# jandrewrfarrell/RUFUS

Hardware: AMD Instinct MI355X
Metric: reads/sec through k-mer count+filter at k=25 (higher is better)
Workload: dtype u64; 1 GPU; synthetic 30x WGS trio (BASELINE configs[2]): genome 3100000000 bp, 620000000/620000000/620000000 x 150 bp reads per sample, on each of 1 GPU(s) 19 resident blocks of the subject (92 GB of packed reads in HBM, generated on the device in 2.7 s), 1000 SNVs, seed 12345, k=25, -s 8G -L 2, MinCov 5, MaxHashDepth 1200, MinQ 15, thresh 1; 2 minimizer-shard pass(es) per step (per-shard (pos,key)-sorted re; parallelism=read-block shard x1, mutant_kmers=24567, pulled_pairs=11560, passes=2, hbm_total=309220868096, hbm_free_at_start=308400881664, resident_read_bytes=92219805240, read_blocks=compact, run_map_budget_bytes=39836680704, checked=False, hbm_mapped_bytes=271656681472

## Files before the change

include/rufus_hip.h:

```cpp
#ifndef RUFUS_HIP_H
#define RUFUS_HIP_H

#include <stddef.h>
#include <stdint.h>

#ifdef __cplusplus
extern "C" {
#endif

#define RFX_OK 0
#define RFX_E_NODEVICE (-1)
#define RFX_E_INVAL (-2)
#define RFX_E_NOMEM (-3)
#define RFX_E_FULL (-4)
#define RFX_E_HIP (-5)
#define RFX_E_MIXEDCASE (-6)
#define RFX_E_RANGE (-7)
#define RFX_E_FORMAT (-8)

#define RFX_HISTO_BINS 10002

typedef struct rfx_ctx rfx_ctx;
typedef struct rfx_reads rfx_reads;
typedef struct rfx_table rfx_table;
// ... 183 lines not shown
rfx_records* rfx_records_load(rfx_ctx*, int k, int lsize, const uint64_t* cols, const void* payload, uint64_t n,
                              int counter_len);
rfx_records* rfx_records_load_fd(rfx_ctx*, int k, int lsize, const uint64_t* cols, int fd, uint64_t offset, uint64_t n,
                                 int counter_len);
rfx_records* rfx_records_from_dev(rfx_ctx*, int k, int lsize, const uint64_t* cols, const uint64_t* d_keys,
                                  const uint32_t* d_counts, uint64_t n);
const uint64_t* rfx_records_dev_keys(const rfx_records*);
const uint32_t* rfx_records_dev_counts(const rfx_records*);
const uint64_t* rfx_records_dev_pos(const rfx_records*);
int rfx_records_histo(const rfx_records*, uint64_t* histo );
int rfx_records_verify(const rfx_records*, uint32_t min_count, uint32_t max_count, uint64_t out[4]);
int rfx_records_checksum(const rfx_records*, uint64_t out[2]);
void rfx_records_free(rfx_records*);

int rfx_merge_unique(rfx_ctx*, const rfx_records* const* files, int n_files, uint32_t min_count, uint64_t* keys_out,
                     uint32_t* counts_out, uint64_t cap, uint64_t* n_out);
int rfx_query(const rfx_records* db, const uint64_t* keys, uint64_t n, uint32_t* counts_out);
int rfx_unique_to_subject(rfx_ctx*, const rfx_records* subject, const rfx_records* const* others, int n_others,
                          uint32_t min_count, uint32_t min_cov, uint32_t max_cov, uint64_t* keys_out,
                          uint32_t* counts_out, uint64_t cap, uint64_t* n_out);
rfx_records* rfx_records_subtract(rfx_ctx*, const rfx_records* a, const rfx_records* const* others, int n_others,
                                  uint32_t min_count, uint32_t max_count);

typedef struct rfx_binned rfx_binned;
typedef struct rfx_candidates rfx_candidates;
rfx_binned* rfx_count_finish_binned(rfx_table*, uint64_t lower, uint64_t upper, uint64_t* histo );
uint64_t rfx_binned_size(const rfx_binned*);
int rfx_binned_bits(const rfx_binned*);
void rfx_binned_free(rfx_binned*);
rfx_candidates* rfx_binned_strike(rfx_ctx*, rfx_binned* subject, const rfx_binned* control, uint32_t min_count,
                                  uint32_t max_count);
int rfx_binned_strike_stats(const rfx_ctx*, uint64_t out[2]);
int rfx_leaf_variant(const rfx_ctx*, int out[2]);
int rfx_candidates_strike(rfx_candidates*, const rfx_binned* control);
uint64_t rfx_candidates_size(const rfx_candidates*);
int rfx_candidates_get(const rfx_candidates*, uint64_t* keys_out);
int rfx_candidates_get_counts(const rfx_candidates*, uint32_t* counts_out);
int rfx_candidates_strike_records(rfx_candidates*, const rfx_records* exclude);
void rfx_candidates_free(rfx_candidates*);
int rfx_binned_get(const rfx_binned*, uint64_t* keys_out, uint32_t* counts_out, uint32_t* bins_out, uint64_t* at_out,
                   uint64_t cap, uint64_t* n_out);
int rfx_binned_checksum(const rfx_binned*, uint64_t out[2]);
int rfx_binned_verify(const rfx_binned*, uint64_t lower, uint64_t upper, uint64_t out[5]);
int rfx_binned_query(const rfx_binned*, const uint64_t* canonical_keys, uint64_t n, uint32_t* counts_out);
const uint64_t* rfx_binned_dev_keys(const rfx_binned*);
const uint32_t* rfx_binned_dev_counts(const rfx_binned*);

rfx_set* rfx_set_build(rfx_ctx*, const uint64_t* fwd_keys, uint64_t n, int k);
uint64_t rfx_set_size(const rfx_set*);
void rfx_set_free(rfx_set*);
int rfx_filter(rfx_set*, const rfx_reads*, int thresh, int last_base_skipped, uint32_t* hits_out,
               uint64_t* hitmask_out, uint64_t* n_hit_reads);
int rfx_filter_many(rfx_set*, const rfx_reads* const* blocks, int n, int thresh, int last_base_skipped,
                    uint64_t* const* hitmask_out, uint64_t* n_hit_reads);

#define RFX_SELECT_READS 0
#define RFX_SELECT_PAIRS 1
rfx_reads* rfx_reads_select(rfx_ctx*, const rfx_reads* src, const uint64_t* hitmask , int mode);
int rfx_reads_origin(const rfx_reads*, uint32_t* block_out, uint32_t* read_out);
rfx_reads* rfx_filter_pull(rfx_set*, const rfx_reads* const* blocks, int n, int thresh, int last_base_skipped, int mode,
                           uint64_t* const* hitmask_out, uint64_t* n_hit_reads);

typedef struct rfx_model_params {
  double sc, stdev, factor, skew, power;
} rfx_model_params;
int rfx_model_residuals(rfx_ctx*, const int64_t* histo, uint32_t n, const rfx_model_params* cand, int n_cand,
// ... 22 lines not shown
```

rufus_amd/capi.py:

```python
from __future__ import annotations

import ctypes as C
import os
import sys

import numpy as np

_HERE = os.path.dirname(os.path.abspath(__file__))
LIB_PATH = os.environ.get("RFX_LIB") or os.path.join(_HERE, "librufus_hip.so")

HISTO_BINS = 10002
PACK_COUNT, PACK_FILTER = 1, 2
COUNT_AUTO, COUNT_TABLE, COUNT_P2L, COUNT_MSP = 0, 1, 2, 3
E_FULL, E_RANGE, E_MIXEDCASE = -4, -7, -6
E_INVAL, E_FORMAT = -2, -8
SELECT_READS, SELECT_PAIRS = 0, 1

u8p, u32p, u64p = C.POINTER(C.c_uint8), C.POINTER(C.c_uint32), C.POINTER(C.c_uint64)

SIGNATURES = {
    "rfx_version": (C.c_char_p, []),
    "rfx_strerror": (C.c_char_p, [C.c_int]),
    "rfx_last_error": (C.c_char_p, []),
    "rfx_jf_matrix": (C.c_int, [C.c_int, C.c_int, u64p]),
    "rfx_jf_pos": (C.c_uint64, [u64p, C.c_int, C.c_int, C.c_uint64]),
    "rfx_pack_words": (C.c_uint64, [u64p, C.c_uint32]),
    "rfx_pack_reads": (C.c_int, [C.c_char_p, C.c_char_p, u64p, C.c_uint32, C.c_int, C.c_int, u64p, u32p, u32p, u32p,
                                 u32p]),
    "rfx_pack_spans": (C.c_int, [C.c_void_p, u64p, u32p, u64p, C.c_uint32, C.c_int, C.c_int, u64p, u32p, u32p, u32p, u32p]),
    "rfx_hashlist_keys": (C.c_long, [C.c_char_p, C.c_size_t, C.c_int, C.c_int, u64p, C.c_size_t]),
    "rfx_jhash_header": (C.c_long, [C.c_int, C.c_int, u64p, C.c_int, C.c_int, C.c_int, C.POINTER(C.c_char_p),
                                    C.c_char_p, C.c_size_t]),
    "rfx_open": (C.c_void_p, [C.c_int, C.c_size_t]),
    "rfx_close": (None, [C.c_void_p]),
    "rfx_sync": (C.c_int, [C.c_void_p]),
    "rfx_host_alloc": (C.c_void_p, [C.c_size_t]),
    "rfx_host_alloc_lazy": (C.c_void_p, [C.c_size_t]),
    "rfx_host_pin": (C.c_int, [C.c_void_p]),
    "rfx_host_cpus": (C.c_uint, []),
    "rfx_host_free": (None, [C.c_void_p]),
    "rfx_stream": (C.c_void_p, [C.c_void_p]),
    "rfx_mem_stats": (C.c_int, [C.c_void_p, u64p, u64p, u64p]),
    "rfx_memcpy_dev": (C.c_int, [C.c_void_p, C.c_void_p, C.c_void_p, C.c_size_t]),
    "rfx_prof_enable": (C.c_int, [C.c_void_p, C.c_int]),
    "rfx_prof_filter": (C.c_int, [C.c_void_p, C.c_char_p]),
    "rfx_prof_reset": (C.c_int, [C.c_void_p]),
    "rfx_prof_query": (C.c_int, [C.c_void_p, C.c_char_p, C.POINTER(C.c_double), u64p]),
    "rfx_prof_names": (C.c_int, [C.c_void_p, C.c_char_p, C.c_size_t]),
    "rfx_reads_device_bytes": (C.c_uint64, [C.c_void_p]),
    "rfx_records_subtract": (C.c_void_p, [C.c_void_p, C.c_void_p, C.POINTER(C.c_void_p), C.c_int, C.c_uint32, C.c_uint32]),
    "rfx_count_finish_binned": (C.c_void_p, [C.c_void_p, C.c_uint64, C.c_uint64, u64p]),
    "rfx_binned_size": (C.c_uint64, [C.c_void_p]),
    "rfx_binned_bits": (C.c_int, [C.c_void_p]),
    "rfx_binned_free": (None, [C.c_void_p]),
    "rfx_binned_strike": (C.c_void_p, [C.c_void_p, C.c_void_p, C.c_void_p, C.c_uint32, C.c_uint32]),
    "rfx_binned_strike_stats": (C.c_int, [C.c_void_p, u64p]),
    "rfx_leaf_variant": (C.c_int, [C.c_void_p, C.POINTER(C.c_int)]),
    "rfx_candidates_strike": (C.c_int, [C.c_void_p, C.c_void_p]),
    "rfx_candidates_size": (C.c_uint64, [C.c_void_p]),
    "rfx_candidates_get": (C.c_int, [C.c_void_p, u64p]),
    "rfx_candidates_free": (None, [C.c_void_p]),
    "rfx_candidates_get_counts": (C.c_int, [C.c_void_p, u32p]),
    "rfx_candidates_strike_records": (C.c_int, [C.c_void_p, C.c_void_p]),
    "rfx_binned_get": (C.c_int, [C.c_void_p, u64p, u32p, u32p, u64p, C.c_uint64, u64p]),
    "rfx_binned_checksum": (C.c_int, [C.c_void_p, u64p]),
    "rfx_binned_verify": (C.c_int, [C.c_void_p, C.c_uint64, C.c_uint64, u64p]),
    "rfx_binned_query": (C.c_int, [C.c_void_p, u64p, C.c_uint64, u32p]),
    "rfx_binned_dev_keys": (C.c_void_p, [C.c_void_p]),
    "rfx_binned_dev_counts": (C.c_void_p, [C.c_void_p]),
    "rfx_reads_upload": (C.c_void_p, [C.c_void_p, u64p, u32p, u32p, u32p, u32p, C.c_uint32]),
    "rfx_reads_free": (None, [C.c_void_p]),
    "rfx_reads_count": (C.c_uint32, [C.c_void_p]),
    "rfx_reads_bases": (C.c_uint64, [C.c_void_p]),
    "rfx_reads_words": (C.c_uint64, [C.c_void_p]),
    "rfx_reads_get": (C.c_int, [C.c_void_p, u64p, u32p, u32p, u32p, u32p]),
    "rfx_tile_plan": (C.c_int, [C.c_uint64, C.c_int, C.c_uint32, u64p, u32p]),
    "rfx_reads_tile": (C.c_void_p, [C.c_void_p, C.c_void_p, C.c_int, C.c_uint32]),
    "rfx_reads_select": (C.c_void_p, [C.c_void_p, C.c_void_p, u64p, C.c_int]),
    "rfx_reads_origin": (C.c_int, [C.c_void_p, u32p, u32p]),
    "rfx_filter_pull": (C.c_void_p, [C.c_void_p, C.POINTER(C.c_void_p), C.c_int, C.c_int, C.c_int, C.c_int, C.POINTER(u64p), u64p]),
    "rfx_synth_reads": (C.c_void_p, [C.c_void_p, C.c_void_p, C.c_uint64, C.c_uint32, C.c_int, C.c_int]),
    "rfx_text_open": (C.c_void_p, [C.c_void_p, C.c_uint64]),
    "rfx_text_close": (None, [C.c_void_p]),
    "rfx_text_room": (C.c_uint64, [C.c_void_p]),
    "rfx_text_bytes": (C.c_uint64, [C.c_void_p]),
    "rfx_text_append": (C.c_long, [C.c_void_p, C.c_char_p, C.c_uint64]),
    "rfx_text_copied": (C.c_int, [C.c_void_p, C.c_long]),
    "rfx_text_wait": (C.c_int, [C.c_void_p, C.c_long]),
    "rfx_text_parse": (C.c_void_p, [C.c_void_p, C.c_int, C.c_int, C.POINTER(C.c_int)]),
    "rfx_text_fetch": (C.c_int, [C.c_void_p, C.c_char_p]),
# ... 968 lines not shown
    def counts(self, raw_keys=None) -> np.ndarray:
        c = np.zeros(len(self), np.uint32)
        _check(lib().rfx_candidates_get_counts(self._h, _p(c, u32p)), "rfx_candidates_get_counts")
        k = self._raw_keys() if raw_keys is None else raw_keys
        return c[k != np.uint64(0xFFFFFFFFFFFFFFFF)]

    def keys_counts(self):
        k = self._raw_keys()
        return k[k != np.uint64(0xFFFFFFFFFFFFFFFF)], self.counts(k)

    def free(self):
        if self._h:
            lib().rfx_candidates_free(self._h)
            self._h = None


def binned_strike(ctx: Context, subject: Binned, control, min_count: int = 0, max_count: int = 0xFFFFFFFF) -> Candidates:
    return Candidates(ctx, lib().rfx_binned_strike(ctx._h, subject._h, control._h if control is not None else None,
                                                   min_count, max_count))


def binned_strike_stats(ctx: Context) -> dict:
    o = np.zeros(2, dtype=np.uint64)
    _check(lib().rfx_binned_strike_stats(ctx._h, _p(o, u64p)), "rfx_binned_strike_stats")
    return {"units": int(o[0]), "deferred": int(o[1])}


def leaf_variant(ctx: Context) -> dict:
    o = np.zeros(2, dtype=np.int32)
    _check(lib().rfx_leaf_variant(ctx._h, o.ctypes.data_as(C.POINTER(C.c_int))), "rfx_leaf_variant")
    return {"kc": int(o[0]), "one": bool(o[1])}


OVL_SAM, OVL_CONTIG, OVL_REGION = 0, 1, 2


def overlap_score(ctx: Context, a: bytes, cands, min_pct: float, min_ovl: int, variant: int = OVL_SAM) -> np.ndarray:
    nb = len(cands)
    arr = (C.c_char_p * max(nb, 1))(*cands)
    lens = (C.c_int * max(nb, 1))(*[len(x) for x in cands])
    out = np.zeros((max(nb, 1), 5), dtype=np.int32)
    _check(lib().rfx_overlap_score(ctx._h, a, len(a), arr, lens, nb, min_pct, min_ovl, variant,
                                   out.ctypes.data_as(C.POINTER(C.c_int))), "rfx_overlap_score")
    return out[:nb]


class OvlPool:

    def __init__(self, ctx: Context, seqs):
        self.ctx, self.n = ctx, len(seqs)
        arr = (C.c_char_p * max(self.n, 1))(*seqs)
        lens = (C.c_int * max(self.n, 1))(*[len(s) for s in seqs])
        self._h = lib().rfx_ovl_pool_create(ctx._h, arr, lens, self.n)
        if not self._h:
            raise RufusError("rfx_ovl_pool_create failed: " + lib().rfx_last_error().decode())

    def set(self, i: int, seq: bytes):
        _check(lib().rfx_ovl_pool_set(self._h, i, seq, len(seq)), "rfx_ovl_pool_set")

    def score(self, cands, min_pct: float, min_ovl: int, variant: int = OVL_SAM, strands: int = 0, query: int | None = None,
              a_explicit: bytes | None = None) -> np.ndarray:
        if (query is None) == (a_explicit is None):
            raise ValueError("give either query (a pool index) or a_explicit (a string)")
        cands = np.ascontiguousarray(cands, dtype=np.int32)
        nb, nstr = len(cands), 2 if strands == 2 else 1
        out = np.zeros((nstr, max(nb, 1), 5), dtype=np.int32)
# ... 93 lines not shown
```

rufus_amd/csrc/rfx_api.hip:

```cpp
#include <algorithm>
#include <condition_variable>
#include <mutex>
#include <cstdio>
#include <cstdlib>
#include <cstring>
#include <sys/mman.h>

#include <atomic>
#include <cerrno>
#include <chrono>
#include <queue>
#include <thread>
#include <vector>

#include <unistd.h>

#include "rfx_internal.h"

namespace {

thread_local char g_err[512] = "";

int hip_fail(hipError_t e, const char* what) {
  snprintf(g_err, sizeof g_err, "%s: %s", what, hipGetErrorString(e));
// ... 2922 lines not shown
      dfree(c, bins);
      dfree(c, counts);
      cap = n;
      continue;
    }
    rfx_candidates* r = new rfx_candidates();
    r->ctx = c;
    r->k = subject->k;
    r->bits = subject->bits;
    r->keys = keys;
    r->bins = bins;
    r->counts = counts;
    r->n = n;
    return r;
  }
  snprintf(g_err, sizeof g_err, "rfx_binned_strike: the candidate list did not converge (internal error)");
  return nullptr;
}

int rfx_binned_strike_stats(const rfx_ctx* c, uint64_t out[2]) {
  if (!c || !out) return RFX_E_INVAL;
  out[0] = c->strike_units;
  out[1] = c->strike_deferred;
  return RFX_OK;
}

int rfx_leaf_variant(const rfx_ctx* c, int out[2]) {
  if (!c || !out) return RFX_E_INVAL;
  out[0] = c->leaf_kc;
  out[1] = c->leaf_kc > 0;
  return RFX_OK;
}

int rfx_candidates_strike(rfx_candidates* a, const rfx_binned* control) {
  if (!a || !control || a->ctx != control->ctx || a->k != control->k) return RFX_E_INVAL;
  rfx_ctx* c = a->ctx;
  (void)hipSetDevice(c->device);
  rfxk::strike_cands(c, a->keys, a->bins, a->n, a->bits, binned_view_of(control));
  HIPCHK(ctx_sync(c));
  return RFX_OK;
}

uint64_t rfx_candidates_size(const rfx_candidates* a) { return a ? a->n : 0; }
int rfx_candidates_get(const rfx_candidates* a, uint64_t* keys_out) {
  if (!a || (a->n && !keys_out)) return RFX_E_INVAL;
  if (!a->n) return RFX_OK;
  (void)hipSetDevice(a->ctx->device);
  HIPCHK(ctx_sync(a->ctx));
  HIPCHK(hipMemcpy(keys_out, a->keys, (size_t)a->n * 8, hipMemcpyDeviceToHost));
  return RFX_OK;
}
int rfx_candidates_get_counts(const rfx_candidates* a, uint32_t* counts_out) {
  if (!a || (a->n && !counts_out)) return RFX_E_INVAL;
  if (!a->n) return RFX_OK;
  (void)hipSetDevice(a->ctx->device);
  HIPCHK(ctx_sync(a->ctx));
  HIPCHK(hipMemcpy(counts_out, a->counts, (size_t)a->n * 4, hipMemcpyDeviceToHost));
  return RFX_OK;
}

int rfx_candidates_strike_records(rfx_candidates* a, const rfx_records* exclude) {
  if (!a || !exclude || a->ctx != exclude->ctx) return RFX_E_INVAL;
  if (a->k != exclude->k) {
    snprintf(g_err, sizeof g_err, "rfx_candidates_strike_records: the records hold %d-mers, the candidates %d-mers", exclude->k, a->k);
    return RFX_E_FORMAT;
  }
// ... 1536 lines not shown
```

rufus_amd/csrc/rfx_internal.h:

```cpp
#pragma once
#include <hip/hip_runtime.h>
#include <stdint.h>

#include <atomic>
#include <map>
#include <string>
#include <vector>

#include "../../include/rufus_hip.h"
#include "rfx_leaf_variant.h"

#define RFX_EMPTY 0xFFFFFFFFFFFFFFFFull
#define RFX_TILE 1024u
#define RFX_TABLE_MARGIN 65536u
#define RFX_PROBE_LIMIT 2048u

struct rfx_prof_span {
  std::string name;
  hipEvent_t e0, e1;
};
struct rfx_prof_acc {
  double ms = 0;
  uint64_t launches = 0;
};
// ... 3 lines not shown
  int ntab = 0;
  uint64_t* lut = nullptr;
  uint64_t* lut_t = nullptr;
  uint64_t* lut_tinv = nullptr;
};

struct rfx_ctx {
  int device = 0;
  hipStream_t stream = nullptr;
  hipStream_t aux = nullptr;
  size_t budget = 0, used = 0;
  int n_cu = 256;
  bool prof = false;
  std::string prof_filter;
  std::vector<rfx_prof_span> spans;
  std::vector<hipEvent_t> free_events;
  std::map<std::string, rfx_prof_acc> acc;
  std::map<void*, size_t> allocs;
  std::multimap<size_t, void*> pool;
  char* arena = nullptr;
  size_t arena_reserved = 0, arena_mapped = 0, arena_gran = 0;
  std::vector<void*> arena_handles;
  std::map<size_t, size_t> arena_free;
  bool arena_off = false;
  size_t peak_used = 0;
  std::vector<int> peer_devices;
  uint32_t lds_opt_in = 0;
  hipError_t launch_error = hipSuccess;
  std::vector<struct rfx_table*> pend_tables;
  double msp_surv_frac[2] = {0, 0};
  uint64_t strike_units = 0, strike_deferred = 0;
  bool strike_by_wave = false;
  int leaf_kc = -1;
  uint64_t bam_stats[4] = {0, 0, 0, 0};
  std::map<uint64_t, double> msp_surv_by_size;
  char* pin = nullptr;
  size_t pin_cap = 0, pin_used = 0;
  uint8_t* load_pin[3] = {nullptr, nullptr, nullptr};
  size_t load_pin_bytes = 0;
  struct pin_read { void* dst; size_t off, n; };
  std::vector<pin_read> pin_reads;
  std::map<std::pair<int, uint64_t>, rfx_hash_consts> consts;
  std::map<int, std::vector<uint64_t>> std_cols;
};

struct rfx_table_stats {
  unsigned long long distinct;
  unsigned int max_disp;
  unsigned int overflow;
};

struct rfx_count_ctl {
  unsigned int ticket;
  unsigned int stop;
  unsigned int lost;
  unsigned int pad;
  unsigned long long ovf_n;
};

struct rfx_table_view {
  uint64_t* keys;
  uint32_t* counts;
  uint64_t slots;
  uint64_t cap;
  int rshift, lshift;
  uint64_t pos_lo, pos_hi;
// ... 418 lines not shown
```

rufus_amd/csrc/rfx_msp.hip:

```cpp
#include <algorithm>
#include <type_traits>

#include "rfx_devutil.h"
#include "rfx_internal.h"

#ifdef RFX_TIMING
__device__ unsigned long long g_tm[2048][32];
#define TM_ROW g_tm[blockIdx.x & 2047u]
#define TM_DECL unsigned long long tm_prev = __builtin_amdgcn_s_memtime()
#define TM(i) do { if (threadIdx.x == 0) { const unsigned long long tm_now = __builtin_amdgcn_s_memtime(); atomicAdd(&TM_ROW[i], tm_now - tm_prev); tm_prev = tm_now; } } while (0)
extern "C" int rfx_debug_timing(unsigned long long* out, int reset) {
  static unsigned long long h[2048][32];
  if (out) {
    if (hipMemcpyFromSymbol(h, HIP_SYMBOL(g_tm), sizeof(g_tm)) != hipSuccess) return -1;
    for (int i = 0; i < 32; ++i) {
      out[i] = 0;
      for (int w = 0; w < 2048; ++w) out[i] += h[w][i];
    }
  }
  if (reset) {
    void* p = nullptr;
    if (hipGetSymbolAddress(&p, HIP_SYMBOL(g_tm)) != hipSuccess || hipMemset(p, 0, sizeof(g_tm)) != hipSuccess) return -1;
  }
  return 0;
// ... 418 lines not shown
  if (SLABS) {
    if (threadIdx.x < P1_BINS) s_slab[2][threadIdx.x] = slab_at(threadIdx.x, pending);
    __syncthreads();
    for (uint32_t i = threadIdx.x; i < 3u * P1_BINS * SLAB; i += blockDim.x) {
      const uint32_t o = i & (SLAB - 1), bw = i >> slab_log2, b = bw & (P1_BINS - 1), which = bw >> 7;
      const uint64_t sb = s_slab[which][b];
      if (sb != ~0ull && (which == 2 || which * SLAB + o >= s_fill[b])) msp_rec12_store(rec_a, sb + o, MSP_EMPTY, 0u);
    }
    __syncthreads();
  }
  if (HMODE == 0 || HMODE == 3) {
    __shared__ uint32_t s_emit;
    if (threadIdx.x == 0) {
      s_maxlen = 0;
      s_emit = 0;
    }
    __syncthreads();
    uint32_t sum = 0;
    for (uint32_t b = threadIdx.x; b < P; b += blockDim.x) {
      const uint32_t v = (s_fine[b >> 1] >> ((b & 1u) * 16)) & 0xFFFFu;
      cnt_rows[(uint64_t)blockIdx.x * P + b] = v;
      sum += v;
    }
    atomicAdd(&s_maxlen, sum);
    atomicAdd(&s_emit, n_emit);
    __syncthreads();
    if (threadIdx.x == 0 && s_maxlen != s_emit) atomicExch(flag, 1u);
  }
  if (HMODE == 1)
    for (uint32_t b = threadIdx.x; b < P; b += blockDim.x) cnt_rows[(uint64_t)blockIdx.x * P + b] = s_fine[b];
}

constexpr int RP_STRIDE = 25;
template <bool CANON, bool QUEUED>
__global__ __launch_bounds__(MP1_BLOCK) void k_msp_replay(rfx_reads_view rv, const uint4* __restrict__ map, int k, int bin_bits,
                                                          uint32_t bin_lo, uint32_t bin_hi, msp_rec12* __restrict__ rec_a,
                                                          uint32_t* __restrict__ coarse_cur, uint32_t cap_a,
                                                          uint32_t* __restrict__ cnt_rows, unsigned int* __restrict__ flag,
                                                          int slab_log2) {
  static_assert(P1_BINS == 128, "the slab bookkeeping below shifts by log2(P1_BINS) = 7");
  __shared__ uint32_t s_fill[P1_BINS];
  __shared__ uint64_t s_slab[3][P1_BINS];
  __shared__ uint32_t s_fine[4096];
  __shared__ uint32_t s_rd[MP1_BLOCK * RP_STRIDE + 4];
  __shared__ uint32_t s_sum, s_emit;
  constexpr int RQ_BATCH = 8, RQ_CAP = 64 * RQ_BATCH;
  __shared__ uint16_t s_q[QUEUED ? MP1_BLOCK / 64 : 1][QUEUED ? RQ_CAP : 1];
  __shared__ uint32_t s_qn[QUEUED ? MP1_BLOCK / 64 : 1];
  const uint32_t P = 1u << bin_bits;
  const int sub_bits = bin_bits - 7;
  const int m = msp_m(k);
  const uint32_t mmask = m >= 16 ? ~0u : (1u << (2 * m)) - 1;
  const uint32_t half_sel = bin_lo >= P / 2 ? 1u : bin_hi <= P / 2 ? 0u : 2u;
  uint32_t n_emit = 0;
  for (uint32_t i = threadIdx.x; i < 4096; i += blockDim.x) s_fine[i] = 0;
  const uint32_t SLAB = 1u << slab_log2;
  constexpr uint32_t P1_NO_SLAB = 0xFFFFFFFFu;
  uint32_t pending = P1_NO_SLAB;
  auto reserve_raw = [&](uint32_t b) -> uint32_t { return atomicAdd(&coarse_cur[b * P1_CUR_STRIDE], SLAB); };
  auto slab_at = [&](uint32_t b, uint32_t at) -> uint64_t {
    if (at == P1_NO_SLAB) return ~0ull;
    if ((uint64_t)at + SLAB > cap_a) {
      atomicExch(flag, 1u);
      return (uint64_t)b * cap_a;
    }
    return (uint64_t)b * cap_a + at;
  };
  if (threadIdx.x < P1_BINS) {
    const bool used = bin_hi > bin_lo && threadIdx.x >= (bin_lo >> sub_bits) && threadIdx.x <= ((bin_hi - 1) >> sub_bits);
    s_fill[threadIdx.x] = 0;
    s_slab[0][threadIdx.x] = used ? slab_at(threadIdx.x, reserve_raw(threadIdx.x)) : ~0ull;
    s_slab[1][threadIdx.x] = used ? slab_at(threadIdx.x, reserve_raw(threadIdx.x)) : ~0ull;
    pending = used ? reserve_raw(threadIdx.x) : P1_NO_SLAB;
  }
  __syncthreads();
  uint32_t* const rd = s_rd + threadIdx.x * RP_STRIDE;
  const uint8_t* const ent8 = (const uint8_t*)(rd + 10);
  const uint8_t* const end8 = (const uint8_t*)(rd + 17);
  const uint32_t n_chunks = (rv.n + MP1_BLOCK - 1) / MP1_BLOCK;
  uint4 nq0 = make_uint4(0, 0, 0, 0), nq1 = make_uint4(0, 0, 0, 31u << 27);
// ... 11 lines not shown
    }
  };
  fetch(blockIdx.x);
  for (uint32_t chunk = blockIdx.x; chunk < n_chunks; chunk += gridDim.x) {
#pragma unroll
    for (int j = 0; j < 5; ++j) {
      uint64_t y = __brevll(nw[4 - j]);
      y = ((y & 0xAAAAAAAAAAAAAAAAull) >> 1) | ((y & 0x5555555555555555ull) << 1);
      rd[2 * j] = (uint32_t)y;
      rd[2 * j + 1] = (uint32_t)(y >> 32);
    }
    const uint32_t q[7] = {nq0.x, nq0.y, nq0.z, nq0.w, nq1.x, nq1.y, nq1.z};
    const uint32_t flags = nq1.w;
    uint32_t cnt = flags >> 27;
    if (cnt == 31u) cnt = 0;
    fetch(chunk + gridDim.x);
    uint32_t gaps = 0, tot = 0;
#pragma unroll
    for (int j = 0; j < 7; ++j) {
      const uint32_t lo = q[j] & 0x0F0F0F0Fu, hi = (q[j] >> 4) & 0x0F0F0F0Fu;
      const uint32_t g = ((lo + 0x01010101u) >> 4) & 0x01010101u;
      const uint32_t gm = (g << 8) - g;
      uint32_t p = ((hi & gm) | (lo & ~gm)) + 0x01010101u;
      p += p << 8;
      p += p << 16;
      p += tot * 0x01010101u;
      tot = p >> 24;
      rd[10 + j] = q[j];
      rd[17 + j] = p;
      gaps |= ((g * 0x01020408u) >> 24) << (4 * j);
    }
    uint32_t mine = ~gaps & ((1u << cnt) - 1u);
    if (half_sel != 2u) mine &= half_sel ? flags : ~flags;
    if constexpr (QUEUED) {
      const uint32_t wv = threadIdx.x >> 6, ln = threadIdx.x & 63u;
      uint16_t* const wq = s_q[wv];
      const uint32_t* const wrd = s_rd + (size_t)(wv * 64u) * RP_STRIDE;
      while (__ballot(mine != 0)) {
        if (ln == 0) s_qn[wv] = 0;
        __builtin_amdgcn_fence(__ATOMIC_ACQ_REL, "wavefront");
        __builtin_amdgcn_wave_barrier();
        uint32_t take = mine;
#pragma unroll
        for (int t = 0; t < RQ_BATCH; ++t) take &= take - 1u;
        take = mine & ~take;
        mine &= ~take;
        uint32_t at = atomicAdd(&s_qn[wv], (uint32_t)__popc(take));
        while (__ballot(take != 0)) {
          if (take) {
            const uint32_t i = (uint32_t)__ffs((int)take) - 1u;
            take &= take - 1u;
            wq[at++] = (uint16_t)(ln | (i << 6));
          }
        }
        __builtin_amdgcn_fence(__ATOMIC_ACQ_REL, "wavefront");
        __builtin_amdgcn_wave_barrier();
        const uint32_t T = s_qn[wv];
        for (uint32_t t0 = 0; t0 < T; t0 += 128u) {
          bool on[2], put[2];
          uint32_t dsc[2], en[2], pe[2], sh[2], d[2][4], run_bin[2], slot[2], bh[2];
          const uint32_t* ord[2];
          uint64_t lo[2];
#pragma unroll
          for (int u = 0; u < 2; ++u) {
            on[u] = t0 + (uint32_t)u * 64u + ln < T;
            dsc[u] = on[u] ? wq[t0 + (uint32_t)u * 64u + ln] : 0u;
          }
// ... 23 lines not shown
              uint32_t y = __brev(~f);
              y = ((y & 0xAAAAAAAAu) >> 1) | ((y & 0x55555555u) << 1);
              c = min(f, y >> (32 - 2 * m));
            }
            bh[u] = msp_binhash(mmer_hash(c));
            run_bin[u] = bh[u] >> (32 - bin_bits);
            put[u] = on[u] && run_bin[u] - bin_lo < bin_hi - bin_lo;
            slot[u] = put[u] ? atomicAdd(&s_fill[run_bin[u] >> sub_bits], 1u) : 0u;
          }
#pragma unroll
          for (int u = 0; u < 2; ++u) {
            if (put[u]) {
              const int n = (int)(en[u] & 15u) + 1;
              const uint32_t back = en[u] >> 4;
              const uint32_t hi = __builtin_amdgcn_alignbit(d[u][3], d[u][2], sh[u]) & 0x3FFFFFu;
              uint64_t w;
              uint32_t x;
              msp_record_make(lo[u], hi, k, n, (uint32_t)(k + n - 1 - m) - back, w, x);
              x |= msp_stamp(bh[u], k);
              const uint32_t coarse = run_bin[u] >> sub_bits;
              if (slot[u] < 2 * SLAB) {
                const uint64_t sb = s_slab[slot[u] >> slab_log2][coarse];
                msp_rec12_store(rec_a, sb + (slot[u] & (SLAB - 1)), w, x);
              } else {
                const uint32_t at2 = atomicAdd(&coarse_cur[coarse * P1_CUR_STRIDE], 1u);
                if (at2 < cap_a) msp_rec12_store(rec_a, (uint64_t)coarse * cap_a + at2, w, x);
                else atomicExch(flag, 1u);
              }
              ++n_emit;
              const uint32_t fb = run_bin[u] - bin_lo;
              atomicAdd(&s_fine[fb >> 2], 1u << ((fb & 3u) * 8));
            }
          }
        }
      }
    } else {
    while (__ballot(mine != 0)) {
      bool on[2];
      uint32_t en[2], pe[2], d[2][4];
#pragma unroll
      for (int u = 0; u < 2; ++u) {
        on[u] = mine != 0;
        const uint32_t i = on[u] ? (uint32_t)__ffs((int)mine) - 1u : 0u;
        mine &= mine - 1u;
        en[u] = ent8[i];
        pe[u] = end8[i];
      }
      uint32_t sh[2];
#pragma unroll
      for (int u = 0; u < 2; ++u) {
        const uint32_t e = (uint32_t)k - 2u + pe[u];
        const uint32_t o = 2u * (159u - e), dw = o >> 5;
        sh[u] = o & 31u;
#pragma unroll
        for (int j = 0; j < 4; ++j) d[u][j] = rd[dw + j];
      }
      uint64_t lo[2];
      uint32_t run_bin[2], slot[2], bh[2];
      bool put[2];
#pragma unroll
      for (int u = 0; u < 2; ++u) {
        const uint32_t back = en[u] >> 4;
        lo[u] = (uint64_t)__builtin_amdgcn_alignbit(d[u][1], d[u][0], sh[u]) |
                ((uint64_t)__builtin_amdgcn_alignbit(d[u][2], d[u][1], sh[u]) << 32);
        const uint32_t f = (uint32_t)(lo[u] >> (2u * back)) & mmask;
        uint32_t c = f;
// ... 1192 lines not shown
  case WL:                                     \
    if (canonical) RFX_MSP_P1_HM(true, WL);    \
    else RFX_MSP_P1_HM(false, WL);             \
    break
  switch (msp_wl(k)) {
    RFX_MSP_P1_WL(11);
    RFX_MSP_P1_WL(12);
    RFX_MSP_P1_WL(13);
    RFX_MSP_P1_WL(14);
    RFX_MSP_P1_WL(15);
    default:
      if (canonical) RFX_MSP_P1_HM(true, MSP_WL_WIDE);
      else RFX_MSP_P1_HM(false, MSP_WL_WIDE);
  }
#undef RFX_MSP_P1_WL
#undef RFX_MSP_P1_HM
#undef RFX_MSP_P1
}

int msp_map_grid(rfx_ctx* c, uint32_t n_reads) {
  const uint32_t chunks = (n_reads + MP1_BLOCK - 1) / MP1_BLOCK;
  return (int)std::max<uint32_t>(8, std::min<uint32_t>((uint32_t)c->n_cu * 3, (chunks + 7) & ~7u));
}

int msp_replay_grid(rfx_ctx* c, uint32_t n_reads) {
  const uint32_t chunks = (n_reads + MP1_BLOCK - 1) / MP1_BLOCK;
  return (int)std::max<uint32_t>(8, std::min<uint32_t>((uint32_t)c->n_cu * 2, (chunks + 7) & ~7u));
}

void msp_replay(rfx_ctx* c, const rfx_reads_view& rv, const void* map, int k, int canonical, int bin_bits, uint32_t bin_lo,
                uint32_t bin_hi, int grid, void* rec_a, uint32_t* coarse_cur, uint32_t cap_a, uint32_t* cnt_rows,
                unsigned int* flag, int slab_log2) {
  rfx_span sp(c, "k_msp_replay");
  static const bool queued = getenv("RFX_REPLAY_OLD") == nullptr;
#define RFX_REPLAY(CANON, Q)                                                                                                  \
  hipLaunchKernelGGL((k_msp_replay<CANON, Q>), dim3(grid), dim3(MP1_BLOCK), 0, c->stream, rv, (const uint4*)map, k, bin_bits, \
                     bin_lo, bin_hi, (msp_rec12*)rec_a, coarse_cur, cap_a, cnt_rows, flag, slab_log2)
  if (canonical) {
    if (queued) RFX_REPLAY(true, true);
    else RFX_REPLAY(true, false);
  } else {
    if (queued) RFX_REPLAY(false, true);
    else RFX_REPLAY(false, false);
  }
#undef RFX_REPLAY
}

void msp_leaf_plan(rfx_ctx* c, uint32_t P, int geo, uint64_t n_records, uint64_t est_survivors, uint32_t extra, uint32_t* grid,
                   uint32_t* chunk, uint32_t* n_chunks) {
  const uint32_t per_cu = geo ? 8 : 4;
  uint64_t g = std::min<uint64_t>(P, (uint64_t)c->n_cu * per_cu);
  g = std::min<uint64_t>(g, std::max<uint64_t>(1, n_records >> 12));
  *grid = (uint32_t)std::max<uint64_t>(g, 1);
  *chunk = MSP_LEAF_CHUNK(geo, n_records >= (1ull << 24));
  const uint64_t per = *chunk - MSP_LEAF_PASS_MAX(geo);
  uint64_t more = (est_survivors + est_survivors / 2) / per + 16 + extra;
  if (getenv("RFX_LEAF_STAGE_TEST")) more = extra;
  *n_chunks = (uint32_t)std::min<uint64_t>((uint64_t)*grid + more, 1u << 30);
}

void msp_leaf(rfx_ctx* c, const uint64_t* const* seg_inst, const uint64_t* const* seg_bs, int nseg,
              const uint64_t* inst0, const uint64_t* bs0, uint32_t P, int k, int canonical, const uint64_t* lut,
              int ntab, int sel_bits, int shift1, uint64_t pos_lo, uint64_t pos_hi, uint64_t lower, uint64_t upper,
              uint64_t* out_w, uint32_t* out_c, uint32_t* cur, uint32_t cap, unsigned int* flag, unsigned int* err,
              unsigned int* stage_short, int geo, const uint32_t* const* seg_ext, const uint32_t* ext0, const msp_stage& st,
              uint32_t launch, uint32_t grid, uint2* bin_at) {
  const int force_mixed = getenv("RFX_LEAF_FORCE_MIXED") != nullptr;
  const int kc = msp_leaf_kc(k, nseg, force_mixed != 0, getenv("RFX_LEAF_GENERIC") != nullptr);
  c->leaf_kc = kc;
  uint32_t* const more = st.more + (bin_at ? 0u : launch);
  {
    rfx_span sp(c, "k_msp_leaf");
#define RFX_MSP_LEAF(CANON, GEO, KC, ONE)                                                                                  \
  hipLaunchKernelGGL((k_msp_leaf<CANON, GEO, KC, ONE>), dim3(grid), dim3(MSP_LEAF_BLK(GEO)), 0, c->stream, seg_inst, seg_bs, \
                     nseg, inst0, bs0, seg_ext, ext0, P, k, lower, upper, st.keys, st.counts, st.chunk, st.fill, more,       \
// ... 174 lines not shown
```

Before: 1.170 billion reads/s.

## Write each wave's replay records in bin order via LDS combine before global store

Adds a COMBINE form of the queued k_msp_replay kernel. The first batches of records are kept in registers, counted per coarse bin with wave-local LDS atomics, scattered into an LDS area sorted by bin, and then written to global memory so that consecutive lanes store contiguous slots. The aim is to coalesce the scattered 12-byte record stores and cut per-record s_fill atomics. In exchange it uses more registers, capped by waves_per_eu 4, and adds extra LDS passes and wave barriers. The form is selected automatically when the bin range spans fewer than 64 coarse bins, and a query API plus a profiling script are added.

```diff
diff --git a/include/rufus_hip.h b/include/rufus_hip.h
--- a/include/rufus_hip.h
+++ b/include/rufus_hip.h
@@ -239,6 +239,7 @@
                                   uint32_t max_count);
 int rfx_binned_strike_stats(const rfx_ctx*, uint64_t out[2]);
 int rfx_leaf_variant(const rfx_ctx*, int out[2]);
+int rfx_replay_variant(const rfx_ctx*, int* out);
 int rfx_candidates_strike(rfx_candidates*, const rfx_binned* control);
 uint64_t rfx_candidates_size(const rfx_candidates*);
 int rfx_candidates_get(const rfx_candidates*, uint64_t* keys_out);
diff --git a/profiles/replay_combine.py b/profiles/replay_combine.py
--- /dev/null
+++ b/profiles/replay_combine.py
@@ -0,0 +1,187 @@
+import argparse
+import csv
+import filecmp
+import glob
+import json
+import os
+import re
+import shutil
+import subprocess
+import sys
+import tempfile
+
+ROOT = os.path.dirname(os.path.dirname(os.path.abspath(__file__)))
+OUT = None
+FLAGS = ["--offload-arch=gfx950", "-O3", "-std=c++17", "-fPIC", "-mllvm", "-amdgpu-atomic-optimizer-strategy=DPP", "--cuda-device-only",
+         "-S", "-Rpass-analysis=kernel-resource-usage"]
+
+
+def say(s):
+    print(s, flush=True)
+    if OUT:
+        OUT.write(s + "\n")
+        OUT.flush()
+
+
+def run(args, cwd, limit, env=None, stderr_to=None):
+    p = subprocess.run(args, cwd=cwd, stdout=subprocess.PIPE, stderr=subprocess.PIPE, timeout=limit, env=dict(os.environ, **(env or {})))
+    if p.returncode != 0:
+        say(f"FAILED rc {p.returncode}: {' '.join(args)} (in {cwd})\n" + p.stderr.decode()[-2000:])
+        raise SystemExit(1)
+    if stderr_to:
+        open(stderr_to, "wb").write(p.stderr)
+    return p.stdout.decode()
+
+
+def bench_line(tree, extra=(), limit=420):
+    return json.loads(run([sys.executable, "bench.py"] + list(extra), tree, limit).strip().splitlines()[-1])
+
+
+def static_rows(tree, label, work):
+    asm, rem = os.path.join(work, label + ".s"), os.path.join(work, label + ".remarks")
+    run(["hipcc"] + FLAGS + [os.path.join(tree, "rufus_amd", "csrc", "rfx_msp.hip"), "-o", asm], tree, 900, stderr_to=rem)
+    usage, name, out = {}, None, {}
+    for ln in open(rem):
+        m = re.search(r"remark: +(Function Name: (\S+)|([A-Za-z ]+?)(?: \[[^\]]*\])?: (\d+))", ln)
+        if m and m.group(2):
+            name = m.group(2)
+        elif m and name:
+            usage.setdefault(name, {})[m.group(3).strip()] = int(m.group(4))
+    for name, body in re.findall(r"^(_Z\w*12k_msp_replayI\w+):[^\n]*\n(.*?)^\.Lfunc_end\d+:", open(asm).read(), re.S | re.M):
+        lines = [re.sub(r"\.L\w+", "L", re.sub(r";.*", "", ln)).strip() for ln in body.splitlines()]
+        lines = [re.sub(r"_Z\w*12k_msp_replayI\w+", "K", ln) for ln in lines if re.match(r"[a-z]+_", ln)]
+        n = {p: sum(ln.startswith(p) for ln in lines) for p in ("v_", "s_", "ds_", "global_", "scratch_")}
+        u = usage.get(name, {})
+        targs = re.search(r"k_msp_replayI((?:Lb[01]E)+)EEv", name).group(1).replace("Lb1E", "true, ").replace("Lb0E", "false, ").rstrip(", ")
+        out[targs] = lines
+        say(f"static    {label:6s} k_msp_replay<{targs}>: VALU {n['v_']}  SALU {n['s_']}  LDS {n['ds_']}  global {n['global_']}  scratch ops "
+            f"{n['scratch_']}  VGPRs {u.get('VGPRs')}  SGPRs {u.get('TotalSGPRs')}  VGPRs spilled {u.get('VGPRs Spill')}  scratch "
+            f"{u.get('ScratchSize')}  waves/SIMD {u.get('Occupancy')}  LDS {u.get('LDS Size')}")
+    return out
+
+
+def sq_row(tree, label, work, genome):
+    d = os.path.join(work, "sq_" + label)
+    ctrs = ("SQ_INSTS_VALU", "SQ_INSTS_SALU", "SQ_INSTS_LDS")
+    run(["rocprofv3", "--pmc", *ctrs, "--output-format", "csv", "-d", d, "-o", "s", "--", sys.executable,
+         "bench.py", "--genome", str(genome), "--passes", "2", "--steps", "1", "--warmup", "1", "--inner"], tree, 600)
+    src = glob.glob(os.path.join(d, "**", "s_counter_collection.csv"), recursive=True)[0]
+    tot, launches = dict.fromkeys(ctrs, 0.0), 0
+    for r in csv.DictReader(open(src)):
+        if re.search(r"k_msp_replay<|12k_msp_replayI", r["Kernel_Name"]) and r["Counter_Name"] in tot:
+            tot[r["Counter_Name"]] += float(r["Counter_Value"])
+            launches += r["Counter_Name"] == "SQ_INSTS_VALU"
+    rows = 2 * 3 * (genome * 30 // 300) * 2 * 150 / 64
+    say(f"sq        {label:6s} k_msp_replay: {launches} launches  rows of 64 bases x passes {rows:.4g}   per row: "
+        + "  ".join(f"{c[9:]} {tot[c] / rows:.2f}" for c in ctrs) + f"   VALU + SALU {(tot[ctrs[0]] + tot[ctrs[1]]) / rows:.2f}")
+    shutil.rmtree(d, ignore_errors=True)
+
+
+SPANS = ("k_msp_part1", "k_msp_map", "k_msp_replay", "k_part2", "k_part3", "k_msp_leaf")
+
+
+def probe_row(tree, label, lib, probe, extra):
+    env = {"RFX_LIB": lib, "RFX_REPLAY_PROBE": str(probe)} if probe else {}
+    p = subprocess.run([sys.executable, "bench.py", "--full", "--no-check", "--no-cpu-baseline"] + extra, cwd=tree, stdout=subprocess.PIPE,
+                       stderr=subprocess.PIPE, timeout=420, env=dict(os.environ, **env))
+    if p.returncode != 0:
+        say(f"FAILED rc {p.returncode}: probe {label}\n" + p.stderr.decode()[-2000:])
+        raise SystemExit(1)
+    ln = json.loads(p.stdout.decode().strip().splitlines()[-1])
+    parts = ln["roofline"]["avg_launch_ms_by_kernel"]
+    late = [x for x in p.stderr.decode().splitlines() if x.startswith("replay_probe")]
+    say(f"probe     {label:8s} " + "  ".join(f"{n} {parts.get(n, 0):.3f}" for n in SPANS) + (f"   {late[-1]}" if late else ""))
+
+
+def main():
+    global OUT
+    ap = argparse.ArgumentParser()
+    ap.add_argument("--parent", default=None)
+    ap.add_argument("--runs", type=int, default=3)
+    ap.add_argument("--only", default="static,kernel,sq,same,headline,pmc")
+    ap.add_argument("--probe-lib", default=None, help="the scratch build of the parent's library with the probes (see above)")
+    ap.add_argument("--pmc-round", default="r19")
+    ap.add_argument("--commit", default="k_msp_replay: a wave's records written in bin order, on top of ef0c7d8")
+    ap.add_argument("--genome", type=int, default=1_000_000_000)
+    ap.add_argument("--out", default=None, help="also append every row to this file")
+    args = ap.parse_args()
+    OUT = open(args.out, "a") if args.out else None
+    only = set(args.only.split(","))
+    parent = os.path.abspath(args.parent) if args.parent else None
+    both = ([("parent", parent)] if parent else []) + [("new", ROOT)]
+    work = tempfile.mkdtemp(prefix="replay_combine_")
+    try:
+        if "probe" in only and args.probe_lib and parent:
+            lib = os.path.abspath(args.probe_lib)
+            for title, extra, seq in (("1 Gb, --passes 2: ms per sample", ["--genome", str(args.genome), "--passes", "2"], (0, 1, 2, 0, 1, 2, 0)),
+                                      ("W: ms per W sample", [], (0, 1, 2, 0))):
+                say("probe     " + title)
+                for pr in seq:
+                    probe_row(parent, ("parent", "probe_a", "probe_b")[pr], lib, pr, extra)
+        if "late" in only and args.probe_lib and parent:
+            probe_row(parent, "count", os.path.abspath(args.probe_lib), 3, ["--genome", str(args.genome), "--passes", "2"])
+        if "static" in only:
+            got = {label: static_rows(tree, label, work) for label, tree in both}
+            if parent:
+                for targs, lines in got["parent"].items():
+                    say(f"static    k_msp_replay<{targs}> of the parent and <{targs}, false> of this build: "
+                        + ("line for line the same" if got["new"].get(targs + ", false") == lines else "DIFFERENT"))
+        if "kernel" in only:
+            for label, tree in both + both[:-1]:
+                ln = bench_line(tree, ["--full", "--no-check", "--no-cpu-baseline"])
+                parts = ln["roofline"]["avg_launch_ms_by_kernel"]
+                say(f"kernel    {label:6s} ms per W sample: " + "  ".join(f"{n} {v:.3f}" for n, v in parts.items())
+                    + f"   chain {ln['roofline']['avg_launch_ms']:.1f}   ms_per_step (brackets on) {ln['ms_per_step']:.1f}")
+        if "headline" in only:
+            ms, facts = {"parent": [], "new": []}, {}
+            for i in range(args.runs):
+                for label, tree in both:
+                    ln = bench_line(tree, ["--no-cpu-baseline"])
+                    ms[label].append(ln["ms_per_step"])
+                    c = ln["config"]
+                    facts[label] = (c["mutant_kmers"], c["pulled_pairs"], c["records_per_sample"], c["hbm_peak_bytes"])
+                    say(f"headline  {label:6s} run {i}: ms_per_step {ln['ms_per_step']:9.3f}   value {ln['value']:.4e} reads/s   mutant_kmers "
+                        f"{c['mutant_kmers']}  pulled_pairs {c['pulled_pairs']}  hbm_peak_bytes {c['hbm_peak_bytes']}")
+            mean = {k: sum(v) / len(v) for k, v in ms.items()}
+            spread = {k: max(v) - min(v) for k, v in ms.items()}
+            gap = mean["parent"] - mean["new"]
+            below = max(ms["new"]) < min(ms["parent"])
+            enough = gap >= 5 * max(spread.values())
+            say(f"headline  means: parent {mean['parent']:.3f}  new {mean['new']:.3f}  gap {gap:.3f} ms ({100 * gap / mean['parent']:.2f} %)   "
+                f"spreads: parent {spread['parent']:.3f}  new {spread['new']:.3f}   every new run below every parent run: {below}   "
+                f"gap >= 5 x larger spread ({5 * max(spread.values()):.3f}): {enough}   -> {'MET' if below and enough else 'NOT MET'}")
+            say(f"headline  results: mutant_kmers / pulled_pairs / records_per_sample equal: {facts['parent'][:3] == facts['new'][:3]}   "
+                f"hbm_peak_bytes new {facts['new'][3]} vs parent {facts['parent'][3]}: "
+                f"{'not above' if facts['new'][3] <= facts['parent'][3] else 'ABOVE'}")
+        if "same" in only:
+            dirs = {}
+            for label, tree in both:
+                dirs[label] = os.path.join(work, "dump_" + label)
+                ln = bench_line(tree, ["--genome", "300000000", "--dump-outputs", dirs[label]])
+                say(f"same      {label:6s} --genome 300000000: mutant_kmers {ln['config']['mutant_kmers']}  pulled_pairs {ln['config']['pulled_pairs']}")
+            for name in ("mutant_keys", "histograms", "records_per_sample", "hit_reads"):
+                a, b = (os.path.join(dirs[x], name + ".npy") for x in ("parent", "new"))
+                same = filecmp.cmp(a, b, shallow=False)
+                say(f"same      {name}.npy: {'byte-identical' if same else 'DIFFERENT'} ({os.path.getsize(b)} bytes)")
+                if not same:
+                    raise SystemExit(1)
+        if "sq" in only:
+            for label, tree in both:
+                sq_row(tree, label, work, args.genome)
+        if "pmc" in only:
+            for ctr, tag in (("FETCH_SIZE", "f"), ("WRITE_SIZE", "w")):
+                run(["rocprofv3", "--pmc", ctr, "--output-format", "csv", "-d", os.path.join(work, "pmc_" + tag), "-o", tag, "--",
+                     sys.executable, "bench.py", "--steps", "1", "--warmup", "0", "--inner"], ROOT, 900)
+                say(f"pmc       {ctr}: collected")
+            f = glob.glob(os.path.join(work, "pmc_f", "**", "f_counter_collection.csv"), recursive=True)[0]
+            w = glob.glob(os.path.join(work, "pmc_w", "**", "w_counter_collection.csv"), recursive=True)[0]
+            js = os.path.join(ROOT, "profiles", f"{args.pmc_round}_pmc_wgs.json")
+            summary = run([sys.executable, os.path.join(ROOT, "profiles", "summarize_pmc.py"), f, w, js, "3", "3100000000"], ROOT, 300,
+                          env={"RFX_COMMIT": args.commit})
+            open(os.path.join(ROOT, "profiles", f"{args.pmc_round}_pmc_summary_wgs.txt"), "w").write(summary)
+            say("pmc       " + summary.splitlines()[0])
+    finally:
+        shutil.rmtree(work, ignore_errors=True)
+
+
+main()
diff --git a/rufus_amd/capi.py b/rufus_amd/capi.py
--- a/rufus_amd/capi.py
+++ b/rufus_amd/capi.py
@@ -56,6 +56,7 @@
     "rfx_binned_strike": (C.c_void_p, [C.c_void_p, C.c_void_p, C.c_void_p, C.c_uint32, C.c_uint32]),
     "rfx_binned_strike_stats": (C.c_int, [C.c_void_p, u64p]),
     "rfx_leaf_variant": (C.c_int, [C.c_void_p, C.POINTER(C.c_int)]),
+    "rfx_replay_variant": (C.c_int, [C.c_void_p, C.POINTER(C.c_int)]),
     "rfx_candidates_strike": (C.c_int, [C.c_void_p, C.c_void_p]),
     "rfx_candidates_size": (C.c_uint64, [C.c_void_p]),
     "rfx_candidates_get": (C.c_int, [C.c_void_p, u64p]),
@@ -1090,6 +1091,15 @@
     return {"kc": int(o[0]), "one": bool(o[1])}
 
 
+REPLAY_OLD, REPLAY_SCATTER, REPLAY_COMBINE = 0, 1, 2
+
+
+def replay_variant(ctx: Context) -> int:
+    o = C.c_int(-1)
+    _check(lib().rfx_replay_variant(ctx._h, C.byref(o)), "rfx_replay_variant")
+    return int(o.value)
+
+
 OVL_SAM, OVL_CONTIG, OVL_REGION = 0, 1, 2
 
 
diff --git a/rufus_amd/csrc/rfx_api.hip b/rufus_amd/csrc/rfx_api.hip
--- a/rufus_amd/csrc/rfx_api.hip
+++ b/rufus_amd/csrc/rfx_api.hip
@@ -2978,6 +2978,12 @@
   return RFX_OK;
 }
 
+int rfx_replay_variant(const rfx_ctx* c, int* out) {
+  if (!c || !out) return RFX_E_INVAL;
+  *out = c->replay_form;
+  return RFX_OK;
+}
+
 int rfx_candidates_strike(rfx_candidates* a, const rfx_binned* control) {
   if (!a || !control || a->ctx != control->ctx || a->k != control->k) return RFX_E_INVAL;
   rfx_ctx* c = a->ctx;
diff --git a/rufus_amd/csrc/rfx_internal.h b/rufus_amd/csrc/rfx_internal.h
--- a/rufus_amd/csrc/rfx_internal.h
+++ b/rufus_amd/csrc/rfx_internal.h
@@ -59,6 +59,7 @@
   uint64_t strike_units = 0, strike_deferred = 0;
   bool strike_by_wave = false;
   int leaf_kc = -1;
+  int replay_form = -1;
   uint64_t bam_stats[4] = {0, 0, 0, 0};
   std::map<uint64_t, double> msp_surv_by_size;
   char* pin = nullptr;
diff --git a/rufus_amd/csrc/rfx_msp.hip b/rufus_amd/csrc/rfx_msp.hip
--- a/rufus_amd/csrc/rfx_msp.hip
+++ b/rufus_amd/csrc/rfx_msp.hip
@@ -474,8 +474,11 @@
 }
 
 constexpr int RP_STRIDE = 25;
-template <bool CANON, bool QUEUED>
-__global__ __launch_bounds__(MP1_BLOCK) void k_msp_replay(rfx_reads_view rv, const uint4* __restrict__ map, int k, int bin_bits,
+constexpr int RC_KEEP = 12, RC_ROUND = 384;
+constexpr int RP_WPE_MIN(bool combine) { return combine ? 4 : 1; }
+constexpr int RP_WPE_MAX(bool combine) { return combine ? 4 : 8; }
+template <bool CANON, bool QUEUED, bool COMBINE = false>
+__global__ __launch_bounds__(MP1_BLOCK) __attribute__((amdgpu_waves_per_eu(RP_WPE_MIN(COMBINE), RP_WPE_MAX(COMBINE)))) void k_msp_replay(rfx_reads_view rv, const uint4* __restrict__ map, int k, int bin_bits,
                                                           uint32_t bin_lo, uint32_t bin_hi, msp_rec12* __restrict__ rec_a,
                                                           uint32_t* __restrict__ coarse_cur, uint32_t cap_a,
                                                           uint32_t* __restrict__ cnt_rows, unsigned int* __restrict__ flag,
@@ -484,10 +487,10 @@
   __shared__ uint32_t s_fill[P1_BINS];
   __shared__ uint64_t s_slab[3][P1_BINS];
   __shared__ uint32_t s_fine[4096];
-  __shared__ uint32_t s_rd[MP1_BLOCK * RP_STRIDE + 4];
+  __shared__ __attribute__((aligned(16))) uint32_t s_rd[MP1_BLOCK * RP_STRIDE + 4];
   __shared__ uint32_t s_sum, s_emit;
   constexpr int RQ_BATCH = 8, RQ_CAP = 64 * RQ_BATCH;
-  __shared__ uint16_t s_q[QUEUED ? MP1_BLOCK / 64 : 1][QUEUED ? RQ_CAP : 1];
+  __shared__ __attribute__((aligned(8))) uint16_t s_q[QUEUED ? MP1_BLOCK / 64 : 1][QUEUED ? RQ_CAP : 1];
   __shared__ uint32_t s_qn[QUEUED ? MP1_BLOCK / 64 : 1];
   const uint32_t P = 1u << bin_bits;
   const int sub_bits = bin_bits - 7;
@@ -565,7 +568,7 @@
     }
     uint32_t mine = ~gaps & ((1u << cnt) - 1u);
     if (half_sel != 2u) mine &= half_sel ? flags : ~flags;
-    if constexpr (QUEUED) {
+    if constexpr (QUEUED && !COMBINE) {
       const uint32_t wv = threadIdx.x >> 6, ln = threadIdx.x & 63u;
       uint16_t* const wq = s_q[wv];
       const uint32_t* const wrd = s_rd + (size_t)(wv * 64u) * RP_STRIDE;
@@ -655,6 +658,197 @@
               atomicAdd(&s_fine[fb >> 2], 1u << ((fb & 3u) * 8));
             }
           }
+        }
+      }
+    } else if constexpr (COMBINE) {
+      static_assert(QUEUED, "COMBINE is a form of the queued kernel");
+      const uint32_t wv = threadIdx.x >> 6, ln = threadIdx.x & 63u;
+      uint16_t* const wq = s_q[wv];
+      const uint32_t* const wrd = s_rd + (size_t)(wv * 64u) * RP_STRIDE;
+      uint64_t kw[RC_KEEP];
+      uint32_t kx[RC_KEEP], km[RC_KEEP / 2];
+#pragma unroll
+      for (int j = 0; j < RC_KEEP / 2; ++j) km[j] = 0xFFFFFFFFu;
+      auto queue_batch = [&]() -> uint32_t {
+        if (ln == 0) s_qn[wv] = 0;
+        __builtin_amdgcn_fence(__ATOMIC_ACQ_REL, "wavefront");
+        __builtin_amdgcn_wave_barrier();
+        uint32_t take = mine;
+#pragma unroll
+        for (int t = 0; t < RQ_BATCH; ++t) take &= take - 1u;
+        take = mine & ~take;
+        mine &= ~take;
+        uint32_t at = atomicAdd(&s_qn[wv], (uint32_t)__popc(take));
+        while (__ballot(take != 0)) {
+          if (take) {
+            const uint32_t i = (uint32_t)__ffs((int)take) - 1u;
+            take &= take - 1u;
+            wq[at++] = (uint16_t)(ln | (i << 6));
+          }
+        }
+        __builtin_amdgcn_fence(__ATOMIC_ACQ_REL, "wavefront");
+        __builtin_amdgcn_wave_barrier();
+        return s_qn[wv];
+      };
+      auto cut2 = [&](uint32_t t0, uint32_t T, auto JC) {
+        constexpr int J = decltype(JC)::value;
+        bool on[2], put[2];
+        uint32_t dsc[2], en[2], pe[2], sh[2], d[2][4], run_bin[2], slot[2], bh[2];
+        const uint32_t* ord[2];
+        uint64_t lo[2];
+#pragma unroll
+        for (int u = 0; u < 2; ++u) {
+          on[u] = t0 + (uint32_t)u * 64u + ln < T;
+          dsc[u] = on[u] ? wq[t0 + (uint32_t)u * 64u + ln] : 0u;
+        }
+#pragma unroll
+        for (int u = 0; u < 2; ++u) {
+          ord[u] = wrd + (size_t)(dsc[u] & 63u) * RP_STRIDE;
+          const uint32_t i = dsc[u] >> 6;
+          en[u] = ((const uint8_t*)(ord[u] + 10))[i];
+          pe[u] = ((const uint8_t*)(ord[u] + 17))[i];
+        }
+#pragma unroll
+        for (int u = 0; u < 2; ++u) {
+          const uint32_t e = (uint32_t)k - 2u + pe[u];
+          const uint32_t o = 2u * (159u - e), dw = o >> 5;
+          sh[u] = o & 31u;
+#pragma unroll
+          for (int j = 0; j < 4; ++j) d[u][j] = ord[u][dw + j];
+        }
+#pragma unroll
+        for (int u = 0; u < 2; ++u) {
+          const uint32_t back = en[u] >> 4;
+          lo[u] = (uint64_t)__builtin_amdgcn_alignbit(d[u][1], d[u][0], sh[u]) |
+                  ((uint64_t)__builtin_amdgcn_alignbit(d[u][2], d[u][1], sh[u]) << 32);
+          const uint32_t f = (uint32_t)(lo[u] >> (2u * back)) & mmask;
+          uint32_t c = f;
+          if (CANON) {
+            uint32_t y = __brev(~f);
+            y = ((y & 0xAAAAAAAAu) >> 1) | ((y & 0x55555555u) << 1);
+            c = min(f, y >> (32 - 2 * m));
+          }
+          bh[u] = msp_binhash(mmer_hash(c));
+          run_bin[u] = bh[u] >> (32 - bin_bits);
+          put[u] = on[u] && run_bin[u] - bin_lo < bin_hi - bin_lo;
+          if constexpr (J < 0) slot[u] = put[u] ? atomicAdd(&s_fill[run_bin[u] >> sub_bits], 1u) : 0u;
+        }
+#pragma unroll
+        for (int u = 0; u < 2; ++u) {
+          if (put[u]) {
+            const int n = (int)(en[u] & 15u) + 1;
+            const uint32_t back = en[u] >> 4;
+            const uint32_t hi = __builtin_amdgcn_alignbit(d[u][3], d[u][2], sh[u]) & 0x3FFFFFu;
+            uint64_t w;
+            uint32_t x;
+            msp_record_make(lo[u], hi, k, n, (uint32_t)(k + n - 1 - m) - back, w, x);
+            x |= msp_stamp(bh[u], k);
+            const uint32_t coarse = run_bin[u] >> sub_bits;
+            if constexpr (J < 0) {
+              if (slot[u] < 2 * SLAB) {
+                const uint64_t sb = s_slab[slot[u] >> slab_log2][coarse];
+                msp_rec12_store(rec_a, sb + (slot[u] & (SLAB - 1)), w, x);
+              } else {
+                const uint32_t at2 = atomicAdd(&coarse_cur[coarse * P1_CUR_STRIDE], 1u);
+                if (at2 < cap_a) msp_rec12_store(rec_a, (uint64_t)coarse * cap_a + at2, w, x);
+                else atomicExch(flag, 1u);
+              }
+            } else {
+              const int S = J + u, SH = (S & 1) * 16;
+              kw[S] = w;
+              kx[S] = x;
+              km[S >> 1] = (km[S >> 1] & ~(0xFFFFu << SH)) | ((coarse - (bin_lo >> sub_bits)) << SH);
+            }
+            ++n_emit;
+            const uint32_t fb = run_bin[u] - bin_lo;
+            atomicAdd(&s_fine[fb >> 2], 1u << ((fb & 3u) * 8));
+          }
+        }
+      };
+      {
+        auto kept_batch = [&](auto BC) {
+          constexpr int B = decltype(BC)::value;
+          const uint32_t T = queue_batch();
+          cut2(0u, T, std::integral_constant<int, 8 * B>());
+          if (T > 128u) cut2(128u, T, std::integral_constant<int, 8 * B + 2>());
+          if constexpr (8 * B + 4 < RC_KEEP) {
+            if (T > 256u) cut2(256u, T, std::integral_constant<int, 8 * B + 4>());
+            if (T > 384u) cut2(384u, T, std::integral_constant<int, 8 * B + 6>());
+          } else {
+            for (uint32_t t0 = 256u; t0 < T; t0 += 128u) cut2(t0, T, std::integral_constant<int, -1>());
+          }
+        };
+        if (__ballot(mine != 0)) kept_batch(std::integral_constant<int, 0>());
+        if (__ballot(mine != 0)) kept_batch(std::integral_constant<int, 1>());
+      }
+      while (__ballot(mine != 0)) {
+        const uint32_t T = queue_batch();
+        for (uint32_t t0 = 0; t0 < T; t0 += 128u) cut2(t0, T, std::integral_constant<int, -1>());
+      }
+      {
+        uint4* const area = (uint4*)(s_rd + (size_t)(wv * 64u) * RP_STRIDE);
+        uint32_t* const cntw = (uint32_t*)(area + RC_ROUND);
+        uint2* const binw = (uint2*)wq;
+        static_assert(4 * RC_ROUND + 64 <= 64 * RP_STRIDE && (64 * RP_STRIDE) % 4 == 0 && 64 * 8 <= 2 * RQ_CAP,
+                      "the sort area is the wave's own");
+        const uint32_t coarse0 = bin_lo >> sub_bits;
+#pragma unroll
+        for (int r = 0; r < 2; ++r) {
+          bool any = false;
+#pragma unroll
+          for (int jj = 0; jj < RC_KEEP / 2; ++jj) {
+            const int S = RC_KEEP / 2 * r + jj;
+            any |= ((km[S >> 1] >> ((S & 1) * 16)) & 0xFFFFu) != 0xFFFFu;
+          }
+          if (!__ballot(any)) continue;
+          cntw[ln] = 0;
+          if (ln == 0) s_qn[wv] = 0;
+          __builtin_amdgcn_fence(__ATOMIC_ACQ_REL, "wavefront");
+          __builtin_amdgcn_wave_barrier();
+#pragma unroll
+          for (int jj = 0; jj < RC_KEEP / 2; ++jj) {
+            const int S = RC_KEEP / 2 * r + jj, SH = (S & 1) * 16;
+            const uint32_t h = (km[S >> 1] >> SH) & 0xFFFFu;
+            if (h != 0xFFFFu) km[S >> 1] |= atomicAdd(&cntw[h], 1u) << (SH + 7);
+          }
+          __builtin_amdgcn_fence(__ATOMIC_ACQ_REL, "wavefront");
+          __builtin_amdgcn_wave_barrier();
+          {
+            const uint32_t cn = cntw[ln];
+            const uint32_t st = atomicAdd(&s_qn[wv], cn);
+            const uint32_t base = cn ? atomicAdd(&s_fill[coarse0 + ln], cn) : 0u;
+            binw[ln] = make_uint2(st, base);
+          }
+          __builtin_amdgcn_fence(__ATOMIC_ACQ_REL, "wavefront");
+          __builtin_amdgcn_wave_barrier();
+          const uint32_t N = s_qn[wv];
+#pragma unroll
+          for (int jj = 0; jj < RC_KEEP / 2; ++jj) {
+            const int S = RC_KEEP / 2 * r + jj, SH = (S & 1) * 16;
+            const uint32_t h = (km[S >> 1] >> SH) & 0xFFFFu;
+            if (h != 0xFFFFu) {
+              const uint32_t lb = h & 127u;
+              const uint2 sb = binw[lb];
+              area[sb.x + (h >> 7)] = make_uint4((uint32_t)kw[S], (uint32_t)(kw[S] >> 32), kx[S], lb << 16 | min(sb.y + (h >> 7), 0xFFFFu));
+            }
+          }
+          __builtin_amdgcn_fence(__ATOMIC_ACQ_REL, "wavefront");
+          __builtin_amdgcn_wave_barrier();
+          for (uint32_t i = ln; i < N; i += 64u) {
+            const uint4 rc = area[i];
+            const uint32_t slot = rc.w & 0xFFFFu, coarse = coarse0 + (rc.w >> 16);
+            const uint64_t w = (uint64_t)rc.x | ((uint64_t)rc.y << 32);
+            if (slot < 2 * SLAB) {
+              const uint64_t sb = s_slab[slot >> slab_log2][coarse];
+              msp_rec12_store(rec_a, sb + (slot & (SLAB - 1)), w, rc.z);
+            } else {
+              const uint32_t at2 = atomicAdd(&coarse_cur[coarse * P1_CUR_STRIDE], 1u);
+              if (at2 < cap_a) msp_rec12_store(rec_a, (uint64_t)coarse * cap_a + at2, w, rc.z);
+              else atomicExch(flag, 1u);
+            }
+          }
+          __builtin_amdgcn_fence(__ATOMIC_ACQ_REL, "wavefront");
+          __builtin_amdgcn_wave_barrier();
         }
       }
     } else {
@@ -1913,15 +2107,20 @@
                 uint32_t bin_hi, int grid, void* rec_a, uint32_t* coarse_cur, uint32_t cap_a, uint32_t* cnt_rows,
                 unsigned int* flag, int slab_log2) {
   rfx_span sp(c, "k_msp_replay");
-  static const bool queued = getenv("RFX_REPLAY_OLD") == nullptr;
-#define RFX_REPLAY(CANON, Q)                                                                                                  \
-  hipLaunchKernelGGL((k_msp_replay<CANON, Q>), dim3(grid), dim3(MP1_BLOCK), 0, c->stream, rv, (const uint4*)map, k, bin_bits, \
-                     bin_lo, bin_hi, (msp_rec12*)rec_a, coarse_cur, cap_a, cnt_rows, flag, slab_log2)
+  const int sub_bits = bin_bits - 7;
+  const bool fits = bin_hi > bin_lo && sub_bits >= 0 && ((bin_hi - 1) >> sub_bits) - (bin_lo >> sub_bits) < 64u;
+  const int form = getenv("RFX_REPLAY_OLD") ? 0 : getenv("RFX_REPLAY_SCATTER") || !fits ? 1 : 2;
+  c->replay_form = form;
+#define RFX_REPLAY(CANON, ...)                                                                                               \
+  hipLaunchKernelGGL((k_msp_replay<CANON, __VA_ARGS__>), dim3(grid), dim3(MP1_BLOCK), 0, c->stream, rv, (const uint4*)map, k, \
+                     bin_bits, bin_lo, bin_hi, (msp_rec12*)rec_a, coarse_cur, cap_a, cnt_rows, flag, slab_log2)
   if (canonical) {
-    if (queued) RFX_REPLAY(true, true);
+    if (form == 2) RFX_REPLAY(true, true, true);
+    else if (form == 1) RFX_REPLAY(true, true);
     else RFX_REPLAY(true, false);
   } else {
-    if (queued) RFX_REPLAY(false, true);
+    if (form == 2) RFX_REPLAY(false, true, true);
+    else if (form == 1) RFX_REPLAY(false, true);
     else RFX_REPLAY(false, false);
   }
 #undef RFX_REPLAY
```

Result: faster. 1.188 billion reads/s (median of 6 runs) (+1.5%).
